# luisdiaz1997/GPzoo

Hardware: AMD Instinct MI355X
Metric: ELBO evals/sec (L=32-latent evaluations, all GPUs) at M=2048 inducing, N=200000, L=32 latents/GPU x 1 GPU(s) (higher is better)
Workload: dtype f32; 1 GPU; BASELINE configs[2]: Slide-seq-shaped synthetic, N=200000 spots, M=2048, L=32 latents/GPU x 1 GPU(s), matern32, f32; latents_total=32, whitened=True, chunk=0, factor_dtype=f64

## Files before the change

gpzoo_amd/build.py:

```python
from __future__ import annotations

import os
import subprocess
import sys

HERE = os.path.dirname(os.path.abspath(__file__))
CSRC = os.path.join(HERE, "csrc")
LIB = os.path.join(HERE, "libgpzoo_hip.so")
SOURCES = ["runtime.hip", "kfill.hip", "gemm.hip", "gemmw.hip", "gemmp.hip", "diag128.hip", "coop.hip", "factor.hip", "kgrad.hip", "mmops.hip", "poisson.hip", "svgp.hip", "vnngp.hip", "collective.hip", "spatial.hip", "nmf.hip", "smooth.hip", "kmeans.hip", "gram.hip", "poisson_sparse.hip", "nmf_sparse.hip", "deviance.hip", "nb.hip", "nb_sparse.hip", "nb_deviance.hip", "gaussian.hip"]
HEADERS = ["common.h", "gemm.h", "cov.h", "gemmw.h", "gemmp.h", "diag128.h", "factor.h", "kgrad.h", "mmops.h", os.path.join("..", "..", "include", "gpzoo_hip.h")]
FLAGS = ["--offload-arch=gfx950", "-O3", "-std=c++17", "-fPIC", "-ffp-contract=fast", "-Wall", "-Wno-unused-function"]
SOURCE_FLAGS = {"spatial.hip": ["-ffp-contract=off"], "smooth.hip": ["-ffp-contract=off"], "kmeans.hip": ["-ffp-contract=off"]}


HASH_MARK = b"GPZ_SRC_HASH:"


def source_hash():
    import hashlib
    h = hashlib.sha256()
    for f in sorted(SOURCES + HEADERS):
        path = os.path.join(CSRC, f)
        if not os.path.exists(path):
            return None
        h.update(os.path.basename(f).encode() + b"\0")
        h.update(open(path, "rb").read())
        h.update(b"\0")
    return h.hexdigest()[:32]


def embedded_hash(lib_path: str = LIB):
    try:
        blob = open(lib_path, "rb").read()
    except OSError:
        return None
    i = blob.find(HASH_MARK)
    if i < 0:
        return None
    j = blob.find(b"\0", i)
    return blob[i + len(HASH_MARK):j].decode("ascii", "replace")


def _stale() -> bool:
    if not os.path.exists(LIB):
        return True
    return embedded_hash() != source_hash()


def build(force: bool = False, verbose: bool = True) -> str:
    if not force and not _stale():
        return LIB
    hipcc = os.environ.get("HIPCC", "/opt/rocm/bin/hipcc")
    objs = []
    procs = []
    for src in SOURCES:
        obj = os.path.join(CSRC, src.replace(".hip", ".o"))
        objs.append(obj)
        extra = [f'-DGPZ_SOURCE_HASH="{source_hash()}"'] if src == "runtime.hip" else []
        extra += SOURCE_FLAGS.get(src, [])
        cmd = [hipcc, *FLAGS, *extra, "-c", os.path.join(CSRC, src), "-o", obj]
        if verbose:
            print(" ".join(cmd), flush=True)
        procs.append((src, subprocess.Popen(cmd, stdout=subprocess.PIPE, stderr=subprocess.STDOUT, text=True)))
    for src, pr in procs:
        out, _ = pr.communicate()
        if pr.returncode != 0:
            raise RuntimeError(f"hipcc failed on {src}:\n{out}")
        if verbose and out.strip():
            print(out)
    cmd = [hipcc, "--offload-arch=gfx950", "-shared", "-fPIC", "-o", LIB, *objs, "-ldl"]
    if verbose:
        print(" ".join(cmd), flush=True)
    subprocess.run(cmd, check=True)
    return LIB


if __name__ == "__main__":
    build(force="--force" in sys.argv)
    print(LIB)
```

gpzoo_amd/csrc/kgrad.hip:

```cpp
#include "kgrad.h"
#include "mmops.h"

namespace gpz {

__device__ __forceinline__ float kg_exp(float x) { return __builtin_amdgcn_exp2f(x * 1.44269504088896341f); }
__device__ __forceinline__ double kg_exp(double x) { return exp(x); }
__device__ __forceinline__ float kg_sqrt(float x) { return sqrtf(x); }
__device__ __forceinline__ double kg_sqrt(double x) { return sqrt(x); }
__device__ __forceinline__ float kg_rsqrt(float x) { return rsqrtf(x); }
__device__ __forceinline__ double kg_rsqrt(double x) { return 1.0 / sqrt(x); }
__device__ __forceinline__ float kg_pow(float x, float y) { return __builtin_amdgcn_exp2f(y * __builtin_amdgcn_logf(x)); }
__device__ __forceinline__ double kg_pow(double x, double y) { return pow(x, y); }

template <typename T, int KIND>
__global__ __launch_bounds__(256) void kgrad_kernel(KgradArgs a) {
  const int l = blockIdx.y, wave = threadIdx.x >> 6, lane = threadIdx.x & 63;
  const int64_t m = (int64_t)blockIdx.x * 4 + wave;
  if (m >= a.M) return;
  const T* kb = static_cast<const T*>(a.Kbar) + (int64_t)l * a.stride + m * a.ld;
  const T* Zp = static_cast<const T*>(a.Z);
  const T* Xp = static_cast<const T*>(a.X);
  const int d = a.d;
  const T sig = static_cast<const T*>(a.sigma)[l];
  const T ell = static_cast<const T*>(a.ell)[l];
  const T s2 = sig * sig, il2 = (T)1 / (ell * ell);
  T z[4] = {0, 0, 0, 0};
  for (int k = 0; k < d; ++k) z[k] = Zp[m * d + k];
  const int gz = (KIND == 2) ? ((uint64_t)a.gZ[m] < (uint64_t)a.G ? (int)a.gZ[m] : 0) : 0;
  const T aeff = (KIND == 2) ? static_cast<const T*>(a.ga)[l] : (T)0;
  const T gpow = (T)a.gpow;
  double dz[4] = {0, 0, 0, 0}, dsig = 0, dell = 0, da = 0;
  constexpr int UN = 4;
  for (int64_t c0 = lane; c0 < a.ncols; c0 += 64 * UN) {
    T g[UN], x[UN][4];
    int gx[UN];
#pragma unroll
    for (int u = 0; u < UN; ++u) {
      const int64_t c = c0 + 64 * u;
      const bool in = c < a.ncols;
      g[u] = in ? kb[c] : (T)0;
#pragma unroll
      for (int k = 0; k < 4; ++k) x[u][k] = (in && k < d) ? Xp[c * d + k] : (T)0;
      gx[u] = (KIND == 2 && in) ? ((uint64_t)a.gX[c] < (uint64_t)a.G ? (int)a.gX[c] : 0) : 0;
    }
    T pz[4] = {0, 0, 0, 0}, psig = 0, pell = 0, pa = 0;
#pragma unroll
    for (int u = 0; u < UN; ++u) {
      T diff[4], d2 = 0;
#pragma unroll
      for (int k = 0; k < 4; ++k) { diff[k] = (k < d) ? z[k] - x[u][k] : (T)0; d2 = fma(diff[k], diff[k], d2); }
      T cz;
      if (KIND == 0) {
        const T kv = s2 * kg_exp((T)-0.5 * d2 * il2);
        psig += g[u] * (T)2 * kv / sig;
        pell += g[u] * kv * d2 * il2 / ell;
        cz = -kv * il2;
      } else if (KIND == 1) {
        const T v = (T)1.7320508075688772935 * kg_sqrt(d2) / ell, e = kg_exp(-v);
        psig += g[u] * (T)2 * sig * ((T)1 + v) * e;
        pell += g[u] * s2 * v * v * e / ell;
        cz = -s2 * (T)3 * il2 * e;
      } else if (KIND == 4) {
        const T rr = kg_sqrt(d2), kv = s2 * kg_exp(-rr / ell);
        psig += g[u] * (T)2 * kv / sig;
        pell += g[u] * kv * rr * il2;
        cz = d2 > (T)0 ? -(kv / ell) * kg_rsqrt(d2) : (T)0;
      } else if (KIND == 5) {
        const T v = (T)2.2360679774997896964 * kg_sqrt(d2) / ell, e = kg_exp(-v), q3 = v * v / (T)3;
        psig += g[u] * (T)2 * sig * ((T)1 + v + q3) * e;
        pell += g[u] * s2 * q3 * ((T)1 + v) * e / ell;
        cz = -s2 * (T)5 / (T)3 * il2 * ((T)1 + v) * e;
      } else {
        const T r2 = static_cast<const T*>(a.gr2)[gz * a.G + gx[u]];
        const T den = aeff * r2 + (T)1;
        const T kv = s2 * kg_exp((T)-0.5 * d2 * il2 / den) * kg_pow(den, -gpow);
        psig += g[u] * (T)2 * kv / sig;
        pell += g[u] * kv * d2 * il2 / (ell * den);
        pa += g[u] * kv * ((T)0.5 * d2 * il2 / (den * den) - gpow / den) * r2;
        cz = -kv * il2 / den;
      }
      const T gc = g[u] * cz;
#pragma unroll
      for (int k = 0; k < 4; ++k) pz[k] = fma(gc, diff[k], pz[k]);
    }
    dsig += (double)psig; dell += (double)pell; da += (double)pa;
#pragma unroll
    for (int k = 0; k < 4; ++k) dz[k] += (double)pz[k];
  }
  double v[7] = {dz[0], dz[1], dz[2], dz[3], dsig * a.scalar_scale, dell * a.scalar_scale, da * a.scalar_scale};
#pragma unroll
  for (int i = 0; i < 7; ++i)
    for (int o = 32; o > 0; o >>= 1) v[i] += __shfl_down(v[i], o);
  if (lane == 0) {
    double* dst = a.acc + ((int64_t)l * a.Mp + m) * 8;
#pragma unroll
    for (int i = 0; i < 7; ++i) dst[i] += v[i];
  }
}

int kgrad_launch(int dtype, int kind, const KgradArgs& a, int L, hipStream_t s) {
  GPZ_REQUIRE((kind >= 0 && kind <= 2) || kind == GPZ_KERNEL_MATERN12 || kind == GPZ_KERNEL_MATERN52,
              "kgrad: unknown kernel kind %d", kind);
  dim3 grid((unsigned)((a.M + 3) / 4), (unsigned)L), block(256);
#define GPZ_KG(T, K) hipLaunchKernelGGL((kgrad_kernel<T, K>), grid, block, 0, s, a)
#define GPZ_KG_KINDS(T) \
  switch (kind) { case 0: GPZ_KG(T, 0); break; case 1: GPZ_KG(T, 1); break; case 4: GPZ_KG(T, 4); break; \
                  case 5: GPZ_KG(T, 5); break; default: GPZ_KG(T, 2); break; }
  if (dtype == GPZ_F32) GPZ_KG_KINDS(float) else GPZ_KG_KINDS(double)
#undef GPZ_KG_KINDS
#undef GPZ_KG
  GPZ_LAUNCH_OK();
  return 0;
}

}

extern "C" size_t gpz_kgrad_workspace_bytes(int64_t nA, int32_t n_latent) {
  if (nA < 1 || n_latent < 1) return 0;
  gpz::Carver c(nullptr);
  c.take<double>((int64_t)n_latent * nA * 8);
  return c.used();
}

extern "C" int gpz_kgrad(const gpz_kernel_desc* k, const void* A, int64_t nA, const void* B, int64_t nB, int32_t d,
                         const int64_t* gA, const int64_t* gB, const void* Kbar, int64_t ldk, int64_t stride_k,
                         double* grad_theta, double* grad_A, void* ws, size_t ws_bytes, void* stream) {
  using namespace gpz;
  GPZ_REQUIRE(k && A && B && Kbar && ws, "gpz_kgrad: null pointer");
  GPZ_REQUIRE(nA >= 1 && nB >= 1 && ldk >= nB && d >= 1 && d <= 4, "gpz_kgrad: bad extents nA=%lld nB=%lld ldk=%lld d=%d",
              (long long)nA, (long long)nB, (long long)ldk, d);
  GPZ_REQUIRE((k->kind >= 0 && k->kind <= 2) || k->kind == GPZ_KERNEL_MATERN12 || k->kind == GPZ_KERNEL_MATERN52,
              "gpz_kgrad: kernel kind %d has no parameters to differentiate", k->kind);
  GPZ_REQUIRE(k->n_latent >= 1 && (k->dtype == GPZ_F32 || k->dtype == GPZ_F64), "gpz_kgrad: bad kernel description");
  if (k->kind == GPZ_KERNEL_MGGP_RBF)
    GPZ_REQUIRE(gA && gB && k->group_a && k->group_r2 && k->n_groups >= 1, "gpz_kgrad: MGGP kernel needs groups, group_a, group_r2");
  GPZ_REQUIRE(ws_bytes >= gpz_kgrad_workspace_bytes(nA, k->n_latent), "gpz_kgrad: workspace too small");
  hipStream_t s = static_cast<hipStream_t>(stream);
  const int L = k->n_latent;
  Carver c(ws);
  double* acc = c.take<double>((int64_t)L * nA * 8);
  GPZ_HIP_OK(hipMemsetAsync(acc, 0, sizeof(double) * L * nA * 8, s));
  KgradArgs a;
  a.Kbar = Kbar; a.ld = ldk; a.stride = stride_k; a.Z = A; a.X = B; a.gZ = gA; a.gX = gB;
  a.sigma = k->sigma; a.ell = k->lengthscale; a.ga = k->group_a; a.gr2 = k->group_r2;
  a.gpow = k->group_pow; a.scalar_scale = 1.0; a.M = nA; a.ncols = nB; a.Mp = nA; a.d = d; a.G = k->n_groups; a.acc = acc;
  if (int rc = kgrad_launch(k->dtype, k->kind, a, L, s)) return rc;
  return kgrad_finish(acc, L, nA, nA, d, nullptr, grad_A, grad_theta, s);
}
```

Baseline: 2.636 ELBO evals/s.

## Add vectorized, double-buffered kgrad kernel specialized on dimension and fast f32 math

Adds a new kernel-gradient kernel, templated on point dimension, that assigns each lane four consecutive columns. It loads Kbar and X with 16-byte vector loads when the pointers are aligned and prefetches the next tile while computing the current one. For f32 non-MGGP kernels it uses precomputed per-latent constants and hardware exp2/rcp intrinsics in place of divisions and sqrt-based formulas. The aim is to cut memory instruction count and ALU cost in the Kbar contraction. The change adds a remainder path for column counts that are not multiples of 256, and keeps the old scalar kernel behind an environment variable.

```diff
diff --git a/gpzoo_amd/build.py b/gpzoo_amd/build.py
--- a/gpzoo_amd/build.py
+++ b/gpzoo_amd/build.py
@@ -8,7 +8,7 @@
 CSRC = os.path.join(HERE, "csrc")
 LIB = os.path.join(HERE, "libgpzoo_hip.so")
 SOURCES = ["runtime.hip", "kfill.hip", "gemm.hip", "gemmw.hip", "gemmp.hip", "diag128.hip", "coop.hip", "factor.hip", "kgrad.hip", "mmops.hip", "poisson.hip", "svgp.hip", "vnngp.hip", "collective.hip", "spatial.hip", "nmf.hip", "smooth.hip", "kmeans.hip", "gram.hip", "poisson_sparse.hip", "nmf_sparse.hip", "deviance.hip", "nb.hip", "nb_sparse.hip", "nb_deviance.hip", "gaussian.hip"]
-HEADERS = ["common.h", "gemm.h", "cov.h", "gemmw.h", "gemmp.h", "diag128.h", "factor.h", "kgrad.h", "mmops.h", os.path.join("..", "..", "include", "gpzoo_hip.h")]
+HEADERS = ["common.h", "gemm.h", "cov.h", "covgrad.h", "gemmw.h", "gemmp.h", "diag128.h", "factor.h", "kgrad.h", "mmops.h", os.path.join("..", "..", "include", "gpzoo_hip.h")]
 FLAGS = ["--offload-arch=gfx950", "-O3", "-std=c++17", "-fPIC", "-ffp-contract=fast", "-Wall", "-Wno-unused-function"]
 SOURCE_FLAGS = {"spatial.hip": ["-ffp-contract=off"], "smooth.hip": ["-ffp-contract=off"], "kmeans.hip": ["-ffp-contract=off"]}
 
diff --git a/gpzoo_amd/csrc/covgrad.h b/gpzoo_amd/csrc/covgrad.h
--- /dev/null
+++ b/gpzoo_amd/csrc/covgrad.h
@@ -0,0 +1,70 @@
+#pragma once
+#include "cov.h"
+
+namespace gpz {
+
+struct CovGradConst { float ce, a, ds0, ds1, ds2, dl, cz; };
+
+template <int KIND>
+__device__ __forceinline__ CovGradConst cov_grad_const(float sigma, float ell) {
+#pragma clang fp contract(off)
+  const CovConst c = cov_const<KIND>(sigma, ell);
+  CovGradConst g;
+  g.ds0 = 2.f * sigma;
+  g.a = g.ds1 = g.ds2 = 0.f;
+  if (KIND == 4) {
+    g.ce = c.c1;
+    g.dl = c.amp / (ell * ell);
+    g.cz = -(c.amp / ell);
+  } else if (KIND == 5) {
+    g.a = 2.2360679774997896964f / ell;
+    g.ce = c.c1;
+    g.ds1 = g.ds0 * g.a;
+    g.ds2 = g.ds0 * ((g.a * g.a) * 0.333333333333333333f);
+    g.dl = c.c2 / ell;
+    g.cz = -c.c2;
+  } else if (KIND == 1) {
+    g.a = 1.7320508075688772935f / ell;
+    g.ce = c.c1;
+    g.ds1 = g.ds0 * g.a;
+    const float s2a2 = c.c0 * g.a;
+    g.dl = s2a2 / ell;
+    g.cz = -s2a2;
+  } else {
+    const float s2il2 = c.amp / (ell * ell);
+    g.ce = c.c0;
+    g.dl = s2il2 / ell;
+    g.cz = -s2il2;
+  }
+  return g;
+}
+
+template <int KIND>
+__device__ __forceinline__ void cov_grad(float d2, const CovGradConst& g, float& ts, float& tl, float& cz) {
+#pragma clang fp contract(off)
+  const float s = cov_radial<KIND>(d2);
+  if (KIND == 4) {
+    const float e = __builtin_amdgcn_exp2f(-(g.ce * s));
+    ts = g.ds0 * e;
+    tl = (g.dl * s) * e;
+    cz = s > 0.f ? (g.cz * e) * __builtin_amdgcn_rcpf(s) : 0.f;
+  } else if (KIND == 5) {
+    const float e = __builtin_amdgcn_exp2f(-(g.ce * s));
+    const float w = __builtin_fmaf(g.a, s, 1.f) * e;
+    ts = __builtin_fmaf(__builtin_fmaf(g.ds2, s, g.ds1), s, g.ds0) * e;
+    tl = (g.dl * d2) * w;
+    cz = g.cz * w;
+  } else if (KIND == 1) {
+    const float e = __builtin_amdgcn_exp2f(-(g.ce * s));
+    ts = __builtin_fmaf(g.ds1, s, g.ds0) * e;
+    tl = (g.dl * d2) * e;
+    cz = g.cz * e;
+  } else {
+    const float e = __builtin_amdgcn_exp2f(g.ce * s);
+    ts = g.ds0 * e;
+    tl = (g.dl * s) * e;
+    cz = g.cz * e;
+  }
+}
+
+}
diff --git a/gpzoo_amd/csrc/kgrad.hip b/gpzoo_amd/csrc/kgrad.hip
--- a/gpzoo_amd/csrc/kgrad.hip
+++ b/gpzoo_amd/csrc/kgrad.hip
@@ -1,3 +1,8 @@
+#include <cstdlib>
+#include <cstring>
+#include <type_traits>
+
+#include "covgrad.h"
 #include "kgrad.h"
 #include "mmops.h"
 
@@ -11,6 +16,43 @@
 __device__ __forceinline__ double kg_rsqrt(double x) { return 1.0 / sqrt(x); }
 __device__ __forceinline__ float kg_pow(float x, float y) { return __builtin_amdgcn_exp2f(y * __builtin_amdgcn_logf(x)); }
 __device__ __forceinline__ double kg_pow(double x, double y) { return pow(x, y); }
+
+template <typename T>
+struct KgLatent { T sig, ell, s2, il2, aeff, gpow; };
+
+template <typename T, int KIND>
+__device__ __forceinline__ T kg_terms(const KgLatent<T>& p, T g, T d2, T r2, T& psig, T& pell, T& pa) {
+  const T sig = p.sig, ell = p.ell, s2 = p.s2, il2 = p.il2;
+  if (KIND == 0) {
+    const T kv = s2 * kg_exp((T)-0.5 * d2 * il2);
+    psig += g * (T)2 * kv / sig;
+    pell += g * kv * d2 * il2 / ell;
+    return -kv * il2;
+  } else if (KIND == 1) {
+    const T v = (T)1.7320508075688772935 * kg_sqrt(d2) / ell, e = kg_exp(-v);
+    psig += g * (T)2 * sig * ((T)1 + v) * e;
+    pell += g * s2 * v * v * e / ell;
+    return -s2 * (T)3 * il2 * e;
+  } else if (KIND == 4) {
+    const T rr = kg_sqrt(d2), kv = s2 * kg_exp(-rr / ell);
+    psig += g * (T)2 * kv / sig;
+    pell += g * kv * rr * il2;
+    return d2 > (T)0 ? -(kv / ell) * kg_rsqrt(d2) : (T)0;
+  } else if (KIND == 5) {
+    const T v = (T)2.2360679774997896964 * kg_sqrt(d2) / ell, e = kg_exp(-v), q3 = v * v / (T)3;
+    psig += g * (T)2 * sig * ((T)1 + v + q3) * e;
+    pell += g * s2 * q3 * ((T)1 + v) * e / ell;
+    return -s2 * (T)5 / (T)3 * il2 * ((T)1 + v) * e;
+  } else {
+    const T aeff = p.aeff, gpow = p.gpow;
+    const T den = aeff * r2 + (T)1;
+    const T kv = s2 * kg_exp((T)-0.5 * d2 * il2 / den) * kg_pow(den, -gpow);
+    psig += g * (T)2 * kv / sig;
+    pell += g * kv * d2 * il2 / (ell * den);
+    pa += g * kv * ((T)0.5 * d2 * il2 / (den * den) - gpow / den) * r2;
+    return -kv * il2 / den;
+  }
+}
 
 template <typename T, int KIND>
 __global__ __launch_bounds__(256) void kgrad_kernel(KgradArgs a) {
@@ -28,7 +70,7 @@
   for (int k = 0; k < d; ++k) z[k] = Zp[m * d + k];
   const int gz = (KIND == 2) ? ((uint64_t)a.gZ[m] < (uint64_t)a.G ? (int)a.gZ[m] : 0) : 0;
   const T aeff = (KIND == 2) ? static_cast<const T*>(a.ga)[l] : (T)0;
-  const T gpow = (T)a.gpow;
+  const KgLatent<T> p = {sig, ell, s2, il2, aeff, (T)a.gpow};
   double dz[4] = {0, 0, 0, 0}, dsig = 0, dell = 0, da = 0;
   constexpr int UN = 4;
   for (int64_t c0 = lane; c0 < a.ncols; c0 += 64 * UN) {
@@ -49,36 +91,8 @@
       T diff[4], d2 = 0;
 #pragma unroll
       for (int k = 0; k < 4; ++k) { diff[k] = (k < d) ? z[k] - x[u][k] : (T)0; d2 = fma(diff[k], diff[k], d2); }
-      T cz;
-      if (KIND == 0) {
-        const T kv = s2 * kg_exp((T)-0.5 * d2 * il2);
-        psig += g[u] * (T)2 * kv / sig;
-        pell += g[u] * kv * d2 * il2 / ell;
-        cz = -kv * il2;
-      } else if (KIND == 1) {
-        const T v = (T)1.7320508075688772935 * kg_sqrt(d2) / ell, e = kg_exp(-v);
-        psig += g[u] * (T)2 * sig * ((T)1 + v) * e;
-        pell += g[u] * s2 * v * v * e / ell;
-        cz = -s2 * (T)3 * il2 * e;
-      } else if (KIND == 4) {
-        const T rr = kg_sqrt(d2), kv = s2 * kg_exp(-rr / ell);
-        psig += g[u] * (T)2 * kv / sig;
-        pell += g[u] * kv * rr * il2;
-        cz = d2 > (T)0 ? -(kv / ell) * kg_rsqrt(d2) : (T)0;
-      } else if (KIND == 5) {
-        const T v = (T)2.2360679774997896964 * kg_sqrt(d2) / ell, e = kg_exp(-v), q3 = v * v / (T)3;
-        psig += g[u] * (T)2 * sig * ((T)1 + v + q3) * e;
-        pell += g[u] * s2 * q3 * ((T)1 + v) * e / ell;
-        cz = -s2 * (T)5 / (T)3 * il2 * ((T)1 + v) * e;
-      } else {
-        const T r2 = static_cast<const T*>(a.gr2)[gz * a.G + gx[u]];
-        const T den = aeff * r2 + (T)1;
-        const T kv = s2 * kg_exp((T)-0.5 * d2 * il2 / den) * kg_pow(den, -gpow);
-        psig += g[u] * (T)2 * kv / sig;
-        pell += g[u] * kv * d2 * il2 / (ell * den);
-        pa += g[u] * kv * ((T)0.5 * d2 * il2 / (den * den) - gpow / den) * r2;
-        cz = -kv * il2 / den;
-      }
+      const T r2 = (KIND == 2) ? static_cast<const T*>(a.gr2)[gz * a.G + gx[u]] : (T)0;
+      const T cz = kg_terms<T, KIND>(p, g[u], d2, r2, psig, pell, pa);
       const T gc = g[u] * cz;
 #pragma unroll
       for (int k = 0; k < 4; ++k) pz[k] = fma(gc, diff[k], pz[k]);
@@ -98,17 +112,159 @@
   }
 }
 
+template <typename T, int N>
+__device__ __forceinline__ void kg_load16(const T* src, T* out) {
+  constexpr int PER = 16 / sizeof(T);
+  static_assert(N % PER == 0, "kg_load16: whole 16-byte pieces only");
+  typedef T V __attribute__((ext_vector_type(PER)));
+#pragma unroll
+  for (int i = 0; i < N / PER; ++i) {
+    const V v = reinterpret_cast<const V*>(src)[i];
+#pragma unroll
+    for (int j = 0; j < PER; ++j) out[i * PER + j] = v[j];
+  }
+}
+
+template <typename T, int D>
+struct KgTrip { T g[4], x[4 * D]; int gx[4]; };
+
+template <typename T, int KIND, int D>
+__global__ __launch_bounds__(256) void kgrad4_kernel(KgradArgs a) {
+  constexpr bool FAST = sizeof(T) == 4 && KIND != 2;
+  const int l = blockIdx.y, lane = threadIdx.x & 63;
+  const int wave = __builtin_amdgcn_readfirstlane((int)(threadIdx.x >> 6));
+  const int64_t m = (int64_t)blockIdx.x * 4 + wave;
+  if (m >= a.M) return;
+  const T* kb = static_cast<const T*>(a.Kbar) + (int64_t)l * a.stride + m * a.ld;
+  const T* Zp = static_cast<const T*>(a.Z);
+  const T* Xp = static_cast<const T*>(a.X);
+  const T* gr2 = static_cast<const T*>(a.gr2);
+  const int64_t* gX = a.gX;
+  const int G = a.G;
+  const int64_t ncols = a.ncols;
+  const T sig = static_cast<const T*>(a.sigma)[l];
+  const T ell = static_cast<const T*>(a.ell)[l];
+  const T aeff = (KIND == 2) ? static_cast<const T*>(a.ga)[l] : (T)0;
+  const KgLatent<T> p = {sig, ell, sig * sig, (T)1 / (ell * ell), aeff, (T)a.gpow};
+  CovGradConst cg = {};
+  if constexpr (FAST) cg = cov_grad_const<KIND>(sig, ell);
+  T z[D];
+#pragma unroll
+  for (int k = 0; k < D; ++k) z[k] = Zp[m * D + k];
+  const int gz = (KIND == 2) ? ((uint64_t)a.gZ[m] < (uint64_t)G ? (int)a.gZ[m] : 0) : 0;
+  double dz[D], dsig = 0, dell = 0, da = 0;
+#pragma unroll
+  for (int k = 0; k < D; ++k) dz[k] = 0;
+
+  auto fetch = [&](auto vec, KgTrip<T, D>& t, int64_t c) {
+    if constexpr (decltype(vec)::value) {
+      kg_load16<T, 4>(kb + c, t.g);
+      kg_load16<T, 4 * D>(Xp + c * D, t.x);
+    } else {
+#pragma unroll
+      for (int u = 0; u < 4; ++u) t.g[u] = kb[c + u];
+#pragma unroll
+      for (int i = 0; i < 4 * D; ++i) t.x[i] = Xp[c * D + i];
+    }
+#pragma unroll
+    for (int u = 0; u < 4; ++u) t.gx[u] = (KIND == 2) ? ((uint64_t)gX[c + u] < (uint64_t)G ? (int)gX[c + u] : 0) : 0;
+  };
+  auto fetch_edge = [&](KgTrip<T, D>& t, int64_t c) {
+#pragma unroll
+    for (int u = 0; u < 4; ++u) {
+      const bool in = c + u < ncols;
+      t.g[u] = in ? kb[c + u] : (T)0;
+#pragma unroll
+      for (int k = 0; k < D; ++k) t.x[u * D + k] = in ? Xp[(c + u) * D + k] : (T)0;
+      t.gx[u] = (KIND == 2 && in) ? ((uint64_t)gX[c + u] < (uint64_t)G ? (int)gX[c + u] : 0) : 0;
+    }
+  };
+  auto contract = [&](const KgTrip<T, D>& t) {
+    T pz[D], psig = 0, pell = 0, pa = 0;
+#pragma unroll
+    for (int k = 0; k < D; ++k) pz[k] = 0;
+#pragma unroll
+    for (int u = 0; u < 4; ++u) {
+      T diff[D], cz;
+#pragma unroll
+      for (int k = 0; k < D; ++k) diff[k] = z[k] - t.x[u * D + k];
+      if constexpr (FAST) {
+        float ts, tl;
+        cov_grad<KIND>(cov_d2<D>(z, t.x + u * D), cg, ts, tl, cz);
+        psig = __builtin_fmaf(t.g[u], ts, psig);
+        pell = __builtin_fmaf(t.g[u], tl, pell);
+      } else {
+        T d2 = 0;
+#pragma unroll
+        for (int k = 0; k < D; ++k) d2 = fma(diff[k], diff[k], d2);
+        const T r2 = (KIND == 2) ? gr2[gz * G + t.gx[u]] : (T)0;
+        cz = kg_terms<T, KIND>(p, t.g[u], d2, r2, psig, pell, pa);
+      }
+      const T gc = t.g[u] * cz;
+#pragma unroll
+      for (int k = 0; k < D; ++k) pz[k] = fma(gc, diff[k], pz[k]);
+    }
+    dsig += (double)psig; dell += (double)pell;
+    if (KIND == 2) da += (double)pa;
+#pragma unroll
+    for (int k = 0; k < D; ++k) dz[k] += (double)pz[k];
+  };
+  const int64_t nfull = ncols >> 8, c_lane = 4 * lane;
+  auto walk = [&](auto vec) {
+    KgTrip<T, D> ta, tb;
+    if (nfull > 0) fetch(vec, ta, c_lane);
+    int64_t t = 0;
+    for (; t + 1 < nfull; t += 2) {
+      fetch(vec, tb, ((t + 1) << 8) + c_lane);
+      contract(ta);
+      if (t + 2 < nfull) fetch(vec, ta, ((t + 2) << 8) + c_lane);
+      contract(tb);
+    }
+    if (t < nfull) contract(ta);
+  };
+  const bool aligned = ((reinterpret_cast<uintptr_t>(kb) | reinterpret_cast<uintptr_t>(Xp)) & 15) == 0;
+  if (aligned) walk(std::true_type{}); else walk(std::false_type{});
+  if (ncols & 255) {
+    KgTrip<T, D> te;
+    fetch_edge(te, (nfull << 8) + c_lane);
+    contract(te);
+  }
+  double v[7] = {0, 0, 0, 0, dsig * a.scalar_scale, dell * a.scalar_scale, da * a.scalar_scale};
+#pragma unroll
+  for (int k = 0; k < D; ++k) v[k] = dz[k];
+#pragma unroll
+  for (int i = 0; i < 7; ++i)
+    for (int o = 32; o > 0; o >>= 1) v[i] += __shfl_down(v[i], o);
+  if (lane == 0) {
+    double* dst = a.acc + ((int64_t)l * a.Mp + m) * 8;
+#pragma unroll
+    for (int i = 0; i < 7; ++i) dst[i] += v[i];
+  }
+}
+
+static bool kgrad_scalar_path() {
+  const char* e = std::getenv("GPZ_KGRAD_PATH");
+  return e && !std::strcmp(e, "scalar");
+}
+
 int kgrad_launch(int dtype, int kind, const KgradArgs& a, int L, hipStream_t s) {
   GPZ_REQUIRE((kind >= 0 && kind <= 2) || kind == GPZ_KERNEL_MATERN12 || kind == GPZ_KERNEL_MATERN52,
               "kgrad: unknown kernel kind %d", kind);
+  GPZ_REQUIRE(a.d >= 1 && a.d <= 4, "kgrad: %d coordinates per point (1..4 supported)", a.d);
   dim3 grid((unsigned)((a.M + 3) / 4), (unsigned)L), block(256);
-#define GPZ_KG(T, K) hipLaunchKernelGGL((kgrad_kernel<T, K>), grid, block, 0, s, a)
+  const bool scalar = kgrad_scalar_path();
+#define GPZ_KG4(T, K, D) hipLaunchKernelGGL((kgrad4_kernel<T, K, D>), grid, block, 0, s, a)
+#define GPZ_KG(T, K)                                                                                       \
+  { if (scalar) { hipLaunchKernelGGL((kgrad_kernel<T, K>), grid, block, 0, s, a); }                       \
+    else switch (a.d) { case 1: GPZ_KG4(T, K, 1); break; case 2: GPZ_KG4(T, K, 2); break;                  \
+                        case 3: GPZ_KG4(T, K, 3); break; default: GPZ_KG4(T, K, 4); break; } }
 #define GPZ_KG_KINDS(T) \
-  switch (kind) { case 0: GPZ_KG(T, 0); break; case 1: GPZ_KG(T, 1); break; case 4: GPZ_KG(T, 4); break; \
-                  case 5: GPZ_KG(T, 5); break; default: GPZ_KG(T, 2); break; }
+  switch (kind) { case 0: GPZ_KG(T, 0) break; case 1: GPZ_KG(T, 1) break; case 4: GPZ_KG(T, 4) break; \
+                  case 5: GPZ_KG(T, 5) break; default: GPZ_KG(T, 2) break; }
   if (dtype == GPZ_F32) GPZ_KG_KINDS(float) else GPZ_KG_KINDS(double)
 #undef GPZ_KG_KINDS
 #undef GPZ_KG
+#undef GPZ_KG4
   GPZ_LAUNCH_OK();
   return 0;
 }
```

After: 2.636 ELBO evals/s. About the same (-0.0%).
